# UBC-AWP/vision-sam3-yolo-lameless

Measured on AMD Instinct MI355X. Metric: frames/sec (whole node) for YOLO+SAM3+DINOv3 feature extraction, 1080p clips, higher is better.
Workload: dtype f16; 1 GPU; BASELINE cfg#5, dense schedule: fused per-frame path on a synthetic 5 s @ 30 fps 1080p clip (150 unique BGR frames resident in HBM): YOLOv8-l detect (letterbox 384x640, NMS, scale_boxes; f16 plan) -> SAM (Hiera-B+ image encoder + FPN at 1024x1024, box-prompted mask decoder, 1080p mask + statistics + contour features) + DINOv3 ViT-L/16 embed (224x224) on EVERY frame; per-frame records packed, gathe; parallelism=one clip per GPU, 1 GPU(s), one gather per step, streams=7

## Files before the change

### vision-sam3-yolo-lameless_amd/csrc/gemm.hip

```cpp
#include "common.h"
#include <stdlib.h>

namespace {

constexpr int BK = 64;

template <int BM, int BN, int AMODE, int OUT_DT>
__global__ __launch_bounds__(256, 2) void gemm_kernel(const lmx_gemm_desc p) {
  extern __shared__ __attribute__((aligned(16))) char smem[];
  half_t* As = reinterpret_cast<half_t*>(smem);
  half_t* Ws = As + 2 * BM * BK;
  constexpr int FM = BM / 32;
  constexpr int FN = BN / 32;
  constexpr int AI = BM / 32;
  constexpr int WI = BN / 32;

  const int tid = threadIdx.x;
  const int lane = tid & 63;
  const int wave = tid >> 6;
  const int wm = wave & 1, wn = wave >> 1;

  const int nwg = gridDim.x;
  const int bid = blockIdx.x;
  const int q = nwg >> 3, r = nwg & 7, xcd = bid & 7;
// ... 69 lines not shown
    half_t* as = As + buf * BM * BK;
    half_t* ws = Ws + buf * BN * BK;
#pragma unroll
    for (int i = 0; i < AI; ++i) {
      const int row = r0 + 32 * i;
      *reinterpret_cast<half8_t*>(as + row * BK + ((c ^ (row & 7)) << 3)) = a_st[i];
    }
#pragma unroll
    for (int i = 0; i < WI; ++i) {
      const int row = r0 + 32 * i;
      *reinterpret_cast<half8_t*>(ws + row * BK + ((c ^ (row & 7)) << 3)) = w_st[i];
    }
  };

  f32x4 acc[FM][FN];
#pragma unroll
  for (int i = 0; i < FM; ++i)
#pragma unroll
    for (int j = 0; j < FN; ++j) acc[i][j] = f32x4{0.f, 0.f, 0.f, 0.f};

  const int nk = (p.K + BK - 1) / BK;
  load_tile(0);
  store_tile(0);
  __syncthreads();

  const int frow = lane & 15;
  const int fq = lane >> 4;
  for (int kt = 0; kt < nk; ++kt) {
    const int buf = kt & 1;
    if (kt + 1 < nk) load_tile(kt + 1);
    const half_t* as = As + buf * BM * BK + (wm * (BM / 2) + frow) * BK;
    const half_t* ws = Ws + buf * BN * BK + (wn * (BN / 2) + frow) * BK;
#pragma unroll
    for (int ks = 0; ks < 2; ++ks) {
      const int coff = (((ks << 2) + fq) ^ (frow & 7)) << 3;
      half8_t af[FM], wf[FN];
#pragma unroll
      for (int i = 0; i < FM; ++i) af[i] = *reinterpret_cast<const half8_t*>(as + i * 16 * BK + coff);
#pragma unroll
      for (int j = 0; j < FN; ++j) wf[j] = *reinterpret_cast<const half8_t*>(ws + j * 16 * BK + coff);
#pragma unroll
      for (int i = 0; i < FM; ++i)
#pragma unroll
        for (int j = 0; j < FN; ++j)
          acc[i][j] = __builtin_amdgcn_mfma_f32_16x16x32_f16(wf[j], af[i], acc[i][j], 0, 0, 0);
    }
    if (kt + 1 < nk) store_tile(buf ^ 1);
    __syncthreads();
  }

  if (p.act == LMX_ACT_SWIGLU) {
    if constexpr (OUT_DT == LMX_F16 && FN % 2 == 0) {
      half_t* C = reinterpret_cast<half_t*>(p.C);
#pragma unroll
      for (int i = 0; i < FM; ++i) {
        const int m = m0 + wm * (BM / 2) + i * 16 + frow;
        if (m >= p.M) continue;
#pragma unroll
        for (int j = 0; j < FN; j += 2) {
          const int n = n0 + wn * (BN / 2) + j * 16 + fq * 4;
          if (n >= p.N) continue;
          f32x4 g = acc[i][j], u = acc[i][j + 1];
          if (p.bias) {
            g += *reinterpret_cast<const f32x4*>(p.bias + n);
            u += *reinterpret_cast<const f32x4*>(p.bias + n + 16);
          }
          const int no = (n >> 5) * 16 + (n & 15);
          f32x4 v;
#pragma unroll
          for (int e = 0; e < 4; ++e) v[e] = __fmul_rn(lmx_act(g[e], LMX_ACT_SILU), u[e]);
          if (p.scale) {
            const f32x4 s = *reinterpret_cast<const f32x4*>(p.scale + no);
#pragma unroll
            for (int e = 0; e < 4; ++e) v[e] = __fmul_rn(v[e], s[e]);
          }
          half4_t o;
#pragma unroll
          for (int e = 0; e < 4; ++e) o[e] = (half_t)v[e];
          *reinterpret_cast<half4_t*>(C + (int64_t)m * p.ldc + no) = o;
        }
      }
    }
    return;
  }

#pragma unroll
  for (int i = 0; i < FM; ++i) {
    const int m = m0 + wm * (BM / 2) + i * 16 + frow;
    if (m >= p.M) continue;
    const int mr = p.res_rows > 0 ? m % p.res_rows : m;
#pragma unroll
    for (int j = 0; j < FN; ++j) {
      const int n = n0 + wn * (BN / 2) + j * 16 + fq * 4;
      if (n >= p.N) continue;
      f32x4 v = acc[i][j];
      if (p.bias) {
        const f32x4 b = *reinterpret_cast<const f32x4*>(p.bias + n);
        v += b;
      }
      if (p.act != LMX_ACT_NONE) {
#pragma unroll
        for (int e = 0; e < 4; ++e) v[e] = lmx_act(v[e], p.act);
      }
      if (p.scale) {
        const f32x4 s = *reinterpret_cast<const f32x4*>(p.scale + n);
#pragma unroll
        for (int e = 0; e < 4; ++e) v[e] = __fmul_rn(v[e], s[e]);
      }
      if (OUT_DT == LMX_F32) {
        float* C = reinterpret_cast<float*>(p.C);
        if (p.res) {
          const f32x4 rr = *reinterpret_cast<const f32x4*>(reinterpret_cast<const float*>(p.res) + (int64_t)mr * p.ldr + n);
#pragma unroll
          for (int e = 0; e < 4; ++e) v[e] = __fadd_rn(v[e], rr[e]);
        }
        *reinterpret_cast<f32x4*>(C + (int64_t)m * p.ldc + n) = v;
      } else {
        half_t* C = reinterpret_cast<half_t*>(p.C);
        if (p.res) {
          const half4_t rr =
              *reinterpret_cast<const half4_t*>(reinterpret_cast<const half_t*>(p.res) + (int64_t)mr * p.ldr + n);
#pragma unroll
          for (int e = 0; e < 4; ++e) v[e] = __fadd_rn((float)(half_t)v[e], (float)rr[e]);
        }
        half4_t o;
#pragma unroll
        for (int e = 0; e < 4; ++e) o[e] = (half_t)v[e];
        *reinterpret_cast<half4_t*>(C + (int64_t)m * p.ldc + n) = o;
      }
    }
  }
}

template <int BM, int BN, int AMODE, int OUT_DT>
int launch(const lmx_gemm_desc& d, hipStream_t st) {
  const int MT = (d.M + BM - 1) / BM, NT = (d.N + BN - 1) / BN;
  const size_t smem = (size_t)2 * (BM + BN) * BK * sizeof(half_t);
  int dev;
  LMX_TRY(lmx_stream_device(st, &dev));
  LMX_TRY(lmx_allow_lds(reinterpret_cast<const void*>(&gemm_kernel<BM, BN, AMODE, OUT_DT>), (int)smem, dev));
  hipLaunchKernelGGL((gemm_kernel<BM, BN, AMODE, OUT_DT>), dim3(MT * NT), dim3(256), smem, st, d);
  return lmx_launch_check("gemm_kernel");
}

template <int AMODE, int OUT_DT>
int dispatch_tile(const lmx_gemm_desc& d, hipStream_t st) {
  if (d.N <= 64 || (d.N < 128 && d.N % 128 != 0)) return launch<128, 64, AMODE, OUT_DT>(d, st);
  return launch<128, 128, AMODE, OUT_DT>(d, st);
}

}

int lmx_gemm2_launch(const lmx_gemm_desc& d, hipStream_t st);

static bool force_v1() {
  static const int v = lmx_env_char("LMX_GEMM_V1");
  return v == '1';
}

extern "C" int lmx_k_gemm(const lmx_gemm_desc* dp, lmx_stream_t stream) {
  LMX_REQUIRE(dp != nullptr, "lmx_k_gemm: null descriptor");
  const lmx_gemm_desc& d = *dp;
  LMX_REQUIRE(d.A && d.W && d.C, "lmx_k_gemm: null A/W/C");
  LMX_REQUIRE(d.M > 0 && d.N > 0 && d.K > 0, "lmx_k_gemm: empty problem M=%d N=%d K=%d", d.M, d.N, d.K);
  LMX_REQUIRE(d.K % 8 == 0, "lmx_k_gemm: K=%d must be a multiple of 8", d.K);
  LMX_REQUIRE(d.N % 4 == 0, "lmx_k_gemm: N=%d must be a multiple of 4", d.N);
  LMX_REQUIRE(d.lda % 8 == 0, "lmx_k_gemm: lda=%lld must be a multiple of 8", (long long)d.lda);
  const bool gated = d.act == LMX_ACT_SWIGLU;
  LMX_REQUIRE(d.ldc % 4 == 0 && d.ldc >= (gated ? d.N / 2 : d.N), "lmx_k_gemm: bad ldc=%lld", (long long)d.ldc);
  LMX_REQUIRE(aligned16(d.A) && aligned16(d.W), "lmx_k_gemm: A/W must be 16-byte aligned");
  LMX_REQUIRE((((uintptr_t)d.C) & 7) == 0, "lmx_k_gemm: C must be 8-byte aligned");
  LMX_REQUIRE(d.out_dtype == LMX_F16 || d.out_dtype == LMX_F32, "lmx_k_gemm: bad out_dtype %d", d.out_dtype);
  LMX_REQUIRE(d.out_dtype == LMX_F16 || aligned16(d.C), "lmx_k_gemm: f32 C must be 16-byte aligned");
  LMX_REQUIRE(d.act >= LMX_ACT_NONE && d.act <= LMX_ACT_SWIGLU, "lmx_k_gemm: bad act %d", d.act);
  if (gated) {
    LMX_REQUIRE(d.N % 32 == 0, "lmx_k_gemm: LMX_ACT_SWIGLU: N=%d (gate + up rows, interleaved by 16) must be a multiple of 32", d.N);
    LMX_REQUIRE(!d.res, "lmx_k_gemm: LMX_ACT_SWIGLU takes no residual");
    LMX_REQUIRE(d.a_mode == 0 && d.a_rep <= 1 && d.split_k <= 1, "lmx_k_gemm: LMX_ACT_SWIGLU: dense A only (a_mode 0; no pooled rows, convolution, a_rep or split_k); a_mode=%d", d.a_mode);
    LMX_REQUIRE(d.out_dtype == LMX_F16, "lmx_k_gemm: LMX_ACT_SWIGLU writes f16 (one rounding of the f32 product)");
  }
  if (d.bias) LMX_REQUIRE(aligned16(d.bias), "lmx_k_gemm: bias must be 16-byte aligned");
  if (d.scale) LMX_REQUIRE(aligned16(d.scale), "lmx_k_gemm: scale must be 16-byte aligned");
  if (d.res) LMX_REQUIRE(d.ldr % 4 == 0 && d.ldr >= d.N, "lmx_k_gemm: bad ldr=%lld", (long long)d.ldr);
  LMX_REQUIRE(d.res_rows >= 0, "lmx_k_gemm: res_rows");
  if (d.a_mode == 0) {
    LMX_REQUIRE(d.a_rep > 1 || d.lda >= d.K, "lmx_k_gemm: lda=%lld < K=%d", (long long)d.lda, d.K);
  } else if (d.a_mode == 1) {
    LMX_REQUIRE(d.Cin > 0 && d.Cin % 8 == 0, "lmx_k_gemm: conv Cin=%d must be a multiple of 8", d.Cin);
    LMX_REQUIRE(d.K == 9 * d.Cin, "lmx_k_gemm: conv K=%d != 9*Cin=%d", d.K, 9 * d.Cin);
    LMX_REQUIRE(d.conv_stride == 1 || d.conv_stride == 2, "lmx_k_gemm: conv stride %d", d.conv_stride);
    LMX_REQUIRE(d.H > 0 && d.W_ > 0, "lmx_k_gemm: conv H/W");
    LMX_REQUIRE(d.Ho == (d.H + 2 - 3) / d.conv_stride + 1 && d.Wo == (d.W_ + 2 - 3) / d.conv_stride + 1,
                "lmx_k_gemm: conv Ho/Wo (%d,%d) inconsistent with H/W (%d,%d) stride %d", d.Ho, d.Wo, d.H, d.W_,
                d.conv_stride);
    LMX_REQUIRE(d.M % (d.Ho * d.Wo) == 0, "lmx_k_gemm: conv M=%d not a multiple of Ho*Wo", d.M);
    LMX_REQUIRE(d.lda >= d.Cin, "lmx_k_gemm: conv pixel stride lda=%lld < Cin=%d", (long long)d.lda, d.Cin);
  } else if (d.a_mode == 2) {
    LMX_REQUIRE(d.lda >= d.K, "lmx_k_gemm: lda=%lld < K=%d", (long long)d.lda, d.K);
    LMX_REQUIRE(d.H > 0 && d.W_ > 0 && d.H % 2 == 0 && d.W_ % 2 == 0 && d.M % (d.H * d.W_) == 0,
                "lmx_k_gemm: pooled rows need an even H x W token grid that divides M (H=%d W=%d M=%d)", d.H, d.W_, d.M);
    LMX_REQUIRE(!d.res && !d.scale && d.act == LMX_ACT_NONE, "lmx_k_gemm: pooled rows: no residual / scale / activation");
    LMX_REQUIRE(((int64_t)d.M * d.lda + d.K) * 2 < 0x7fffffffll, "lmx_k_gemm: pooled rows: A must be smaller than 2 GB");
    LMX_REQUIRE(d.M >= 512 && d.N >= 96 && d.N % 8 == 0 && d.ldc % 8 == 0 && aligned16(d.C),
                "lmx_k_gemm: pooled rows are built for the LDS-DMA kernel (M >= 512, N >= 96, N %% 8 == 0): use GEMM + maxpool2 for M=%d N=%d", d.M, d.N);
  } else {
    LMX_REQUIRE(false, "lmx_k_gemm: bad a_mode %d", d.a_mode);
  }
  LMX_REQUIRE(d.a_rep >= 0 && d.a_rep <= 3, "lmx_k_gemm: a_rep=%d (0..3)", d.a_rep);
  LMX_REQUIRE(d.split_k >= 0 && d.split_k <= 64, "lmx_k_gemm: split_k=%d (0..64)", d.split_k);
  if (d.split_k > 1) {
    LMX_REQUIRE(d.out_dtype == LMX_F32 && d.act == LMX_ACT_NONE && d.a_mode != 2 && d.a_rep <= 1, "lmx_k_gemm: split_k needs f32 output, no activation, a_mode 0 or 1");
    LMX_REQUIRE(d.split_stride >= (int64_t)(d.M - 1) * d.ldc + d.N && d.split_stride % 4 == 0, "lmx_k_gemm: split_stride=%lld", (long long)d.split_stride);
    LMX_REQUIRE((d.K + 63) / 64 >= d.split_k, "lmx_k_gemm: split_k=%d exceeds the k-tiles of K=%d", d.split_k, d.K);
    const bool conv_ok2 = d.a_mode == 1 && d.Cin % 32 == 0 && d.H < 32768 && d.W_ < 32768;
    LMX_REQUIRE((d.a_mode == 0 || conv_ok2) && d.N >= 64 && d.N % 8 == 0 && d.ldc % 8 == 0 && (!d.res || d.ldr % 8 == 0) &&
                    aligned16(d.C) && (!d.res || aligned16(d.res)),
                "lmx_k_gemm: split_k is built into the LDS-DMA kernel only (N >= 64, N %% 8 == 0; conv: Cin %% 32 == 0); M=%d N=%d", d.M, d.N);
    return lmx_gemm2_launch(d, reinterpret_cast<hipStream_t>(stream));
  }
  if (d.a_rep > 1) {
    LMX_REQUIRE(d.a_mode == 0 && d.K % d.a_rep == 0 && (d.K / d.a_rep) % 64 == 0, "lmx_k_gemm: a_rep=%d needs a_mode 0 and K / a_rep a multiple of 64 (K=%d)", d.a_rep, d.K);
    LMX_REQUIRE(d.lda >= d.K / d.a_rep, "lmx_k_gemm: lda=%lld < K / a_rep", (long long)d.lda);
    LMX_REQUIRE(d.M >= 512 && d.N >= 96 && d.N % 8 == 0 && d.ldc % 8 == 0 && (!d.res || d.ldr % 8 == 0) && aligned16(d.C) && (!d.res || aligned16(d.res)),
                "lmx_k_gemm: a_rep is built into the LDS-DMA kernel only (M >= 512, N >= 96, N %% 8 == 0); M=%d N=%d", d.M, d.N);
    return lmx_gemm2_launch(d, reinterpret_cast<hipStream_t>(stream));
  }
  hipStream_t st = reinterpret_cast<hipStream_t>(stream);
  const bool conv_ok = d.a_mode == 1 && d.Cin % 32 == 0 && d.H < 32768 && d.W_ < 32768;
  if (d.a_mode == 2) return lmx_gemm2_launch(d, st);
  static const int n64 = lmx_env_char("LMX_GEMM_N64") != '0';
  const int n_min = (conv_ok && n64 && d.M >= 65536) ? 64 : 96;
  if ((d.a_mode == 0 || conv_ok) && d.M >= 512 && d.N >= n_min && d.N % 8 == 0 && d.ldc % 8 == 0 && (!d.res || d.ldr % 8 == 0) &&
      aligned16(d.C) && (!d.res || aligned16(d.res)) && !force_v1())
    return lmx_gemm2_launch(d, st);
  if (d.a_mode == 0) {
    return d.out_dtype == LMX_F16 ? dispatch_tile<0, LMX_F16>(d, st) : dispatch_tile<0, LMX_F32>(d, st);
  }
  return d.out_dtype == LMX_F16 ? dispatch_tile<1, LMX_F16>(d, st) : dispatch_tile<1, LMX_F32>(d, st);
}
```

### vision-sam3-yolo-lameless_amd/csrc/gemm2.hip

```cpp
#include "common.h"
#include <stdlib.h>
#include <type_traits>

#ifdef LMX_DBG_TIMELINE
__device__ unsigned long long lmx_tl[8 * 16384];
extern "C" int lmx_dbg_get_timeline(void* host, int64_t bytes) { return (int)hipMemcpyFromSymbol(host, HIP_SYMBOL(lmx_tl), bytes); }
#define TL(i, v) if (threadIdx.x == 0 && swz < 16384) lmx_tl[swz * 8 + (i)] = (v)
#else
#define TL(i, v)
#endif
namespace lmx_gemm2 {

__device__ __forceinline__ float act_apply(float v, int act) { return lmx_act(v, act); }

constexpr int smem_bytes(int BM, int BN, int BK, int NSTAGE) { return NSTAGE * (BM + BN) * BK * 2 + 2 * BN * 4; }
constexpr int waves_per_simd(int BM, int BN, int BK, int NSTAGE) {
  const int smem = smem_bytes(BM, BN, BK, NSTAGE), nwave = (BM / 64) * (BN / 64);
  const int wps = (smem <= 80 * 1024 ? 2 : 1) * nwave / 4;
  return wps < 1 ? 1 : wps;
}
template <int OUT_DT, int BM, int BN, int BK, int NSTAGE, int AMODE, int STAG, bool GATED = false>
__global__ __launch_bounds__(waves_per_simd(BM, BN, BK, NSTAGE) * 256) void gemm2_kernel(const lmx_gemm_desc p, const int ntiles, const int nt_ok) {
  constexpr int NWAVE = (BM / 64) * (BN / 64);
  constexpr int STAGE_BYTES = (BM + BN) * BK * 2;
  constexpr int A_INSTR = BM * BK * 2 / 1024 / NWAVE;
  constexpr int W_INSTR = BN * BK * 2 / 1024 / NWAVE;
  constexpr int ROWS_PER_INSTR = 1024 / (BK * 2);
  constexpr int CHUNKS = BK / 8;
  constexpr int LA = NSTAGE - 1;
  extern __shared__ __attribute__((aligned(16))) char smem[];
  const int tid = threadIdx.x;
  const int lane = tid & 63;
  const int wave = __builtin_amdgcn_readfirstlane(tid >> 6);
  const int wm = wave % (BM / 64), wn = wave / (BM / 64);

  const int bid = blockIdx.x, xcd = bid & 7;
  const int q = ntiles >> 3, r = ntiles & 7;
  const int base = xcd < r ? xcd * (q + 1) : r * (q + 1) + (xcd - r) * q;
  const int cnt = q + (xcd < r ? 1 : 0);
  const int stride = ((int)gridDim.x + 7 - xcd) >> 3;
  const int NT = (p.N + BN - 1) / BN;
  for (int li = bid >> 3; li < cnt; li += stride) {
  const int swz = base + li;
  const int S_ = p.split_k > 1 ? p.split_k : 1;
  const int tile_ = swz / S_, sp_ = swz - tile_ * S_;
  const int mt = tile_ / NT, nt = tile_ - mt * NT;
  const int m0 = mt * BM, n0 = nt * BN;
  TL(0, (unsigned long long)__builtin_amdgcn_s_getreg((31 << 11) | 4));
  TL(1, (unsigned long long)__builtin_amdgcn_s_getreg((31 << 11) | 20));
  TL(2, wall_clock64());
  TL(5, (unsigned long long)bid);

  const int hw_out = (AMODE == 1) ? p.Ho * p.Wo : 1;
  const int img0 = (AMODE == 1) ? m0 / hw_out : 0;
  const char* Ab = reinterpret_cast<const char*>(p.A) +
                   ((AMODE == 1) ? (int64_t)img0 * p.H * p.W_ * p.lda * 2 : (AMODE == 2 ? (int64_t)0 : (int64_t)m0 * p.lda * 2));
  const char* Wb = reinterpret_cast<const char*>(p.W) + (int64_t)n0 * p.K * 2;
  const int Ka = (AMODE == 0 && p.a_rep > 1) ? p.K / p.a_rep : p.K;
  int64_t a_bytes = (AMODE == 1) ? ((int64_t)(p.M / hw_out - img0) * p.H * p.W_ - 1) * p.lda * 2 + (int64_t)p.Cin * 2
                                 : ((int64_t)(p.M - (AMODE == 2 ? 0 : m0) - 1) * p.lda + Ka) * 2;
  int64_t w_bytes = (int64_t)(p.N - n0) * p.K * 2;
  if (a_bytes > 0x7FFFFFF0ll) a_bytes = 0x7FFFFFF0ll;
  if (w_bytes > 0x7FFFFFF0ll) w_bytes = 0x7FFFFFF0ll;
  const __amdgpu_buffer_rsrc_t a_rs = __builtin_amdgcn_make_buffer_rsrc(const_cast<char*>(Ab), 0, (int)a_bytes, 0x00020000);
  const __amdgpu_buffer_rsrc_t w_rs = __builtin_amdgcn_make_buffer_rsrc(const_cast<char*>(Wb), 0, (int)w_bytes, 0x00020000);

  const int lrow = lane / CHUNKS;
  const int lsw = (BK == 64) ? (lrow & 7) : ((-(lrow >> 2)) & 3);
  const int lchunk = (lane % CHUNKS) ^ lsw;
  unsigned a_off[A_INSTR], w_off[W_INSTR];
  int a_yx[A_INSTR];
#pragma unroll
  for (int j = 0; j < A_INSTR; ++j) {
    const int row = (wave * A_INSTR + j) * ROWS_PER_INSTR + lrow;
    if (AMODE == 0) {
      a_off[j] = (unsigned)(row * (int)p.lda * 2 + lchunk * 16);
      a_yx[j] = 0;
    } else if (AMODE == 2) {
      const int m = m0 + row, g = m >> 2, sub = m & 3;
      const int Wq = p.W_ >> 1, gpi = (p.H >> 1) * Wq;
      const int img = g / gpi, rem = g - img * gpi;
      const int gy = rem / Wq, gx = rem - gy * Wq;
      const int tok = (img * p.H + 2 * gy + (sub >> 1)) * p.W_ + 2 * gx + (sub & 1);
      a_off[j] = m < p.M ? (unsigned)(tok * (int)p.lda * 2 + lchunk * 16) : 0x80000000u;
      a_yx[j] = 0;
    } else {
      const int m = m0 + row;
      const int img = m / hw_out, rem = m - img * hw_out;
      const int oy = rem / p.Wo, ox = rem - oy * p.Wo;
      const int iy0 = oy * p.conv_stride - 1, ix0 = ox * p.conv_stride - 1;
      a_off[j] = (unsigned)((((img - img0) * p.H + iy0) * p.W_ + ix0) * (int)p.lda * 2 + lchunk * 16);
      a_yx[j] = (m < p.M) ? ((iy0 << 16) | (ix0 & 0xffff)) : 0x80008000;
    }
  }
#pragma unroll
  for (int j = 0; j < W_INSTR; ++j)
    w_off[j] = (unsigned)(((wave * W_INSTR + j) * ROWS_PER_INSTR + lrow) * p.K * 2 + lchunk * 16);
  const unsigned OOB = 0x80000000u;
  const int nk = (p.K + BK - 1) / BK;
  const int nk64 = (p.K + 63) / 64;
  const int kt0 = (int)((int64_t)sp_ * nk64 / S_) * (64 / BK);
  const int kte = sp_ + 1 == S_ ? nk : (int)((int64_t)(sp_ + 1) * nk64 / S_) * (64 / BK);
  const int nloc = kte - kt0;
  const int nkA = (AMODE == 0 && p.a_rep > 1) ? nk / p.a_rep : nk;
  const bool k_tail_lane = (nk - 1) * BK + lchunk * 8 >= p.K;

  auto issue = [&](int kt, int slot) {
    char* st = smem + slot * STAGE_BYTES;
    const bool kill = (kt == nk - 1) && k_tail_lane;
    const int soff = kt * (BK * 2);
    if (AMODE != 1) {
      const int kta = kt - (kt >= nkA ? nkA : 0) - (kt >= 2 * nkA ? nkA : 0);
      const int soff_a = (AMODE == 0) ? kta * (BK * 2) : soff;
#pragma unroll
      for (int j = 0; j < A_INSTR; ++j) {
        char* dst = st + (wave * A_INSTR + j) * 1024;
        lds_dma16(a_rs, dst, kill ? OOB : a_off[j], soff_a);
      }
    } else {
      const int k0 = kt * BK;
      const int tap = k0 / p.Cin, ci0 = k0 - tap * p.Cin;
      const int ky = tap / 3, kx = tap - 3 * ky;
      const int tap_off = ((ky * p.W_ + kx) * (int)p.lda + ci0) * 2;
#pragma unroll
      for (int j = 0; j < A_INSTR; ++j) {
        char* dst = st + (wave * A_INSTR + j) * 1024;
        const int iy = (a_yx[j] >> 16) + ky, ix = (int)(short)(a_yx[j] & 0xffff) + kx;
        const bool ok = (unsigned)iy < (unsigned)p.H && (unsigned)ix < (unsigned)p.W_;
        lds_dma16(a_rs, dst, ok ? a_off[j] + (unsigned)tap_off : OOB, 0);
      }
    }
#pragma unroll
    for (int j = 0; j < W_INSTR; ++j) {
      char* dst = st + BM * BK * 2 + (wave * W_INSTR + j) * 1024;
      lds_dma16(w_rs, dst, kill ? OOB : w_off[j], soff);
    }
  };

  f32x4 acc[4][4];
#pragma unroll
  for (int i = 0; i < 4; ++i)
#pragma unroll
    for (int j = 0; j < 4; ++j) acc[i][j] = f32x4{0.f, 0.f, 0.f, 0.f};

  float* bl = reinterpret_cast<float*>(smem + NSTAGE * STAGE_BYTES);
  float bias_v = 0.f, scale_v = 1.f;
  if (AMODE != 1 && tid < BN && n0 + tid < p.N) {
    if (p.bias && sp_ == 0) bias_v = p.bias[n0 + tid];
    if constexpr (GATED) {
      if (p.scale && tid < BN / 2 && (n0 >> 1) + tid < (p.N >> 1)) scale_v = p.scale[(n0 >> 1) + tid];
    } else {
      if (p.scale) scale_v = p.scale[n0 + tid];
    }
  }

#pragma unroll
  for (int t = 0; t < LA; ++t)
    if (t < nloc) issue(kt0 + t, t);

  const int frow = lane & 15, fq = lane >> 4;
  const int fsw = (BK == 64) ? (frow & 7) : ((-(frow >> 2)) & 3);
  constexpr int PT = A_INSTR + W_INSTR;
  if constexpr (STAG == 0) {
  for (int kt = 0; kt < nloc; ++kt) {
    const int left = nloc - 1 - kt;
    wait_tiles<PT>(left < LA - 1 ? left : LA - 1);
    __builtin_amdgcn_s_barrier();
#ifdef LMX_DBG_TIMELINE
    if (kt == 0) { TL(6, wall_clock64()); }
    if (kt == 1) { TL(7, wall_clock64()); }
#endif
    if (kt + LA < nloc) issue(kt0 + kt + LA, (kt + LA) % NSTAGE);
    const char* st = smem + (kt % NSTAGE) * STAGE_BYTES;
    const half_t* as = reinterpret_cast<const half_t*>(st) + (wm * 64 + frow) * BK;
    const half_t* ws = reinterpret_cast<const half_t*>(st + BM * BK * 2) + (wn * 64 + frow) * BK;
#ifdef LMX_DBG_NOMFMA
    if (p.M < 0)
#endif
#pragma unroll
    for (int ks = 0; ks < BK / 32; ++ks) {
      const int coff = (((ks << 2) + fq) ^ fsw) << 3;
      half8_t af[4], wf[4];
#pragma unroll
      for (int j = 0; j < 4; ++j) wf[j] = *reinterpret_cast<const half8_t*>(ws + j * 16 * BK + coff);
#pragma unroll
      for (int i = 0; i < 4; ++i) af[i] = *reinterpret_cast<const half8_t*>(as + i * 16 * BK + coff);
      __builtin_amdgcn_s_setprio(1);
#pragma unroll
      for (int i = 0; i < 4; ++i)
#pragma unroll
        for (int j = 0; j < 4; ++j)
          acc[i][j] = __builtin_amdgcn_mfma_f32_16x16x32_f16(wf[j], af[i], acc[i][j], 0, 0, 0);
      __builtin_amdgcn_s_setprio(0);
    }
  }
  } else {
  const int grp = wave >= NWAVE / 2 ? 1 : 0;
  {
    const int y = nloc - 1 < LA - 1 ? nloc - 1 : LA - 1;
    wait_tiles<PT>(y);
  }
  __builtin_amdgcn_s_barrier();
  if (grp) __builtin_amdgcn_s_barrier();
  for (int kt = 0; kt < nloc; ++kt) {
    const char* st = smem + (kt % NSTAGE) * STAGE_BYTES;
    const half_t* as = reinterpret_cast<const half_t*>(st) + (wm * 64 + frow) * BK;
    const half_t* ws = reinterpret_cast<const half_t*>(st + BM * BK * 2) + (wn * 64 + frow) * BK;
    half8_t af[BK / 32][4], wf[BK / 32][4];
#pragma unroll
    for (int ks = 0; ks < BK / 32; ++ks) {
      const int coff = (((ks << 2) + fq) ^ fsw) << 3;
#pragma unroll
      for (int j = 0; j < 4; ++j) wf[ks][j] = *reinterpret_cast<const half8_t*>(ws + j * 16 * BK + coff);
#pragma unroll
      for (int i = 0; i < 4; ++i) af[ks][i] = *reinterpret_cast<const half8_t*>(as + i * 16 * BK + coff);
    }
    if (kt + 1 < nloc) {
      const int rest = nloc - 2 - kt;
      wait_tiles<PT>(rest < LA - 2 ? (rest < 0 ? 0 : rest) : (LA - 2 < 0 ? 0 : LA - 2));
    }
    if (kt + LA < nloc) issue(kt0 + kt + LA, (kt + LA) % NSTAGE);
    asm volatile("s_waitcnt lgkmcnt(0)" ::: "memory");
    __builtin_amdgcn_s_barrier();
    __builtin_amdgcn_s_setprio(1);
#pragma unroll
    for (int ks = 0; ks < BK / 32; ++ks)
#pragma unroll
      for (int i = 0; i < 4; ++i)
#pragma unroll
        for (int j = 0; j < 4; ++j)
          acc[i][j] = __builtin_amdgcn_mfma_f32_16x16x32_f16(wf[ks][j], af[ks][i], acc[i][j], 0, 0, 0);
    __builtin_amdgcn_s_setprio(0);
    __builtin_amdgcn_s_barrier();
  }
  if (!grp) __builtin_amdgcn_s_barrier();
  }

  if (AMODE == 1 && tid < BN && n0 + tid < p.N) {
    if (p.bias && sp_ == 0) bias_v = p.bias[n0 + tid];
    if (p.scale) scale_v = p.scale[n0 + tid];
  }
  if (tid < BN) {
    bl[tid] = bias_v;
    bl[BN + tid] = scale_v;
  }
  asm volatile("s_waitcnt lgkmcnt(0)" ::: "memory");
  __builtin_amdgcn_s_barrier();
  TL(3, wall_clock64());
#ifdef LMX_DBG_NOEPI
  if (p.M > 0 && acc[0][0][0] != 12345.f) continue;
#endif
  const bool nt_out = nt_ok && OUT_DT == LMX_F16 && ((p.ldc * 2) & 127) == 0 && (int64_t)p.M * p.N >= (16ll << 20);
  char* my = smem + wave * 4608;
  auto epilogue = [&](auto act_c, auto scale_c) {
    constexpr int ACT = decltype(act_c)::value;
    constexpr bool SCALE = decltype(scale_c)::value;
    const float* blj = bl + wn * 64 + fq * 4;
    auto finish = [&](f32x4 v, int j) -> f32x4 {
      v += *reinterpret_cast<const f32x4*>(blj + j * 16);
      if constexpr (ACT == LMX_ACT_GELU) {
        const f32x2 g0 = gelu_pk(f32x2{v[0], v[1]}), g1 = gelu_pk(f32x2{v[2], v[3]});
        v = f32x4{g0[0], g0[1], g1[0], g1[1]};
      } else if constexpr (ACT != LMX_ACT_NONE) {
#pragma unroll
        for (int e = 0; e < 4; ++e) v[e] = act_apply(v[e], ACT);
      }
      if constexpr (SCALE) v *= *reinterpret_cast<const f32x4*>(blj + BN + j * 16);
      return v;
    };
    if constexpr (ACT == LMX_ACT_SWIGLU) {
      if constexpr (OUT_DT == LMX_F16 && AMODE == 0) {
        half_t* t16 = reinterpret_cast<half_t*>(my);
        constexpr int RS = 40;
        const bool nt_g = nt_ok && ((p.ldc * 2) & 127) == 0 && (int64_t)p.M * p.N >= (32ll << 20);
#pragma unroll
        for (int pass = 0; pass < 2; ++pass) {
#pragma unroll
          for (int ii = 0; ii < 2; ++ii)
#pragma unroll
            for (int jj = 0; jj < 2; ++jj) {
              const f32x4 g = acc[pass * 2 + ii][2 * jj] + *reinterpret_cast<const f32x4*>(blj + jj * 32);
              const f32x4 u = acc[pass * 2 + ii][2 * jj + 1] + *reinterpret_cast<const f32x4*>(blj + jj * 32 + 16);
              f32x4 v;
#pragma unroll
              for (int e = 0; e < 4; ++e) v[e] = __fmul_rn(act_apply(g[e], LMX_ACT_SILU), u[e]);
              if constexpr (SCALE) {
                const f32x4 sc = *reinterpret_cast<const f32x4*>(bl + BN + wn * 32 + jj * 16 + fq * 4);
#pragma unroll
                for (int e = 0; e < 4; ++e) v[e] = __fmul_rn(v[e], sc[e]);
              }
              const half4_t o = {(half_t)v[0], (half_t)v[1], (half_t)v[2], (half_t)v[3]};
              *reinterpret_cast<half4_t*>(t16 + (ii * 16 + frow) * RS + jj * 16 + fq * 4) = o;
            }
#pragma unroll
          for (int it = 0; it < 2; ++it) {
            const int row = it * 16 + (lane >> 2), c8 = lane & 3;
            const half8_t o = *reinterpret_cast<const half8_t*>(t16 + row * RS + c8 * 8);
            const int m = m0 + wm * 64 + pass * 32 + row;
            const int no = ((n0 + wn * 64) >> 1) + c8 * 8;
            if (m < p.M && no < (p.N >> 1)) {
              half8_t* dst = reinterpret_cast<half8_t*>(reinterpret_cast<half_t*>(p.C) + (int64_t)m * p.ldc + no);
              if (nt_g)
                asm volatile("global_store_dwordx4 %0, %1, off nt" ::"v"(dst), "v"(o) : "memory");
              else
                *dst = o;
            }
          }
        }
      }
    } else if constexpr (OUT_DT == LMX_F16 && AMODE == 2) {
#pragma unroll
      for (int pass = 0; pass < 4; ++pass)
#pragma unroll
        for (int j = 0; j < 4; ++j) {
          f32x4 v = finish(acc[pass][j], j);
#pragma unroll
          for (int e = 0; e < 4; ++e) {
            v[e] = fmaxf(v[e], __shfl_xor(v[e], 1, 64));
            v[e] = fmaxf(v[e], __shfl_xor(v[e], 2, 64));
          }
          const int m = m0 + wm * 64 + pass * 16 + frow;
          const int n = n0 + wn * 64 + j * 16 + fq * 4;
          if ((frow & 3) == 0 && m < p.M && n < p.N)
            *reinterpret_cast<half4_t*>(reinterpret_cast<half_t*>(p.C) + (int64_t)(m >> 2) * p.ldc + n) =
                half4_t{(half_t)v[0], (half_t)v[1], (half_t)v[2], (half_t)v[3]};
          __builtin_amdgcn_sched_barrier(0);
        }
    } else if constexpr (OUT_DT == LMX_F16) {
      half_t* t16 = reinterpret_cast<half_t*>(my);
      constexpr int RS = 72;
#pragma unroll
      for (int pass = 0; pass < 2; ++pass) {
#pragma unroll
        for (int ii = 0; ii < 2; ++ii)
#pragma unroll
          for (int j = 0; j < 4; ++j) {
            const f32x4 v = finish(acc[pass * 2 + ii][j], j);
            const half4_t o = {(half_t)v[0], (half_t)v[1], (half_t)v[2], (half_t)v[3]};
            *reinterpret_cast<half4_t*>(t16 + (ii * 16 + frow) * RS + j * 16 + fq * 4) = o;
          }
#pragma unroll
        for (int it = 0; it < 4; ++it) {
          const int row = it * 8 + (lane >> 3), c8 = lane & 7;
          half8_t o = *reinterpret_cast<const half8_t*>(t16 + row * RS + c8 * 8);
          const int m = m0 + wm * 64 + pass * 32 + row;
          const int n = n0 + wn * 64 + c8 * 8;
          if (m < p.M && n < p.N) {
            if (p.res) {
              const int mr = p.res_rows > 0 ? m % p.res_rows : m;
              const half8_t rr = *reinterpret_cast<const half8_t*>(reinterpret_cast<const half_t*>(p.res) + (int64_t)mr * p.ldr + n);
#pragma unroll
              for (int e = 0; e < 8; ++e) o[e] = (half_t)((float)o[e] + (float)rr[e]);
            }
            half8_t* dst = reinterpret_cast<half8_t*>(reinterpret_cast<half_t*>(p.C) + (int64_t)m * p.ldc + n);
            if (nt_out)
              asm volatile("global_store_dwordx4 %0, %1, off nt" ::"v"(dst), "v"(o) : "memory");
            else
              *dst = o;
          }
        }
      }
    } else if constexpr (AMODE == 2) {
#pragma unroll
      for (int pass = 0; pass < 4; ++pass)
#pragma unroll
        for (int j = 0; j < 4; ++j) {
          f32x4 v = finish(acc[pass][j], j);
#pragma unroll
          for (int e = 0; e < 4; ++e) {
            v[e] = fmaxf(v[e], __shfl_xor(v[e], 1, 64));
            v[e] = fmaxf(v[e], __shfl_xor(v[e], 2, 64));
          }
          const int m = m0 + wm * 64 + pass * 16 + frow;
          const int n = n0 + wn * 64 + j * 16 + fq * 4;
          if ((frow & 3) == 0 && m < p.M && n < p.N) *reinterpret_cast<f32x4*>(reinterpret_cast<float*>(p.C) + (int64_t)(m >> 2) * p.ldc + n) = v;
          __builtin_amdgcn_sched_barrier(0);
        }
    } else {
      float* t32 = reinterpret_cast<float*>(my);
      constexpr int RS = 68;
      const int lrow = lane >> 4, c16 = lane & 15;
      const int n = n0 + wn * 64 + c16 * 4;
      const bool has_res = p.res != nullptr && sp_ == 0;
      float* Cs = reinterpret_cast<float*>(p.C) + (int64_t)sp_ * p.split_stride;
      f32x4 rr[4];
      auto load_res = [&](int pass) {
        f32x4* d = rr;
#pragma unroll
        for (int it = 0; it < 4; ++it) {
          const int m = m0 + wm * 64 + pass * 16 + it * 4 + lrow;
          d[it] = f32x4{0.f, 0.f, 0.f, 0.f};
          if (has_res && m < p.M && n < p.N) {
            const int mr = p.res_rows > 0 ? m % p.res_rows : m;
            d[it] = *reinterpret_cast<const f32x4*>(reinterpret_cast<const float*>(p.res) + (int64_t)mr * p.ldr + n);
          }
        }
      };
#pragma unroll
      for (int pass = 0; pass < 4; ++pass) {
        load_res(pass);
#pragma unroll
        for (int j = 0; j < 4; ++j) *reinterpret_cast<f32x4*>(t32 + frow * RS + j * 16 + fq * 4) = finish(acc[pass][j], j);
#pragma unroll
        for (int it = 0; it < 4; ++it) {
          const int row = it * 4 + lrow;
          f32x4 o = *reinterpret_cast<const f32x4*>(t32 + row * RS + c16 * 4);
          const int m = m0 + wm * 64 + pass * 16 + row;
          if (m < p.M && n < p.N) {
            if (has_res) o += rr[it];
            *reinterpret_cast<f32x4*>(Cs + (int64_t)m * p.ldc + n) = o;
          }
        }
      }
    }
  };
  {
    using T = std::true_type;
    using F = std::false_type;
    const int act = p.act;
    if constexpr (GATED) {
      if (p.scale) epilogue(std::integral_constant<int, LMX_ACT_SWIGLU>{}, T{});
      else epilogue(std::integral_constant<int, LMX_ACT_SWIGLU>{}, F{});
    } else if (p.scale) {
      if (act == LMX_ACT_NONE) epilogue(std::integral_constant<int, LMX_ACT_NONE>{}, T{});
      else if (act == LMX_ACT_SILU) epilogue(std::integral_constant<int, LMX_ACT_SILU>{}, T{});
      else if (act == LMX_ACT_GELU) epilogue(std::integral_constant<int, LMX_ACT_GELU>{}, T{});
      else epilogue(std::integral_constant<int, LMX_ACT_RELU>{}, T{});
    } else {
      if (act == LMX_ACT_NONE) epilogue(std::integral_constant<int, LMX_ACT_NONE>{}, F{});
      else if (act == LMX_ACT_SILU) epilogue(std::integral_constant<int, LMX_ACT_SILU>{}, F{});
      else if (act == LMX_ACT_GELU) epilogue(std::integral_constant<int, LMX_ACT_GELU>{}, F{});
      else epilogue(std::integral_constant<int, LMX_ACT_RELU>{}, F{});
    }
  }
  __builtin_amdgcn_s_barrier();
  TL(4, wall_clock64());
  }
}

template <int BM, int BN, int BK, int NSTAGE, int AMODE, int STAG = 0>
int launch2(const lmx_gemm_desc& d, hipStream_t st) {
  const int MT = (d.M + BM - 1) / BM, NT = (d.N + BN - 1) / BN;
  const size_t smem = smem_bytes(BM, BN, BK, NSTAGE);
  int dev;
  LMX_TRY(lmx_stream_device(st, &dev));
  LMX_TRY(lmx_allow_lds(reinterpret_cast<const void*>(&gemm2_kernel<LMX_F16, BM, BN, BK, NSTAGE, AMODE, STAG>), (int)smem, dev));
  LMX_TRY(lmx_allow_lds(reinterpret_cast<const void*>(&gemm2_kernel<LMX_F32, BM, BN, BK, NSTAGE, AMODE, STAG>), (int)smem, dev));
  const int ntiles = MT * NT * (d.split_k > 1 ? d.split_k : 1);
  int grid = ntiles;
  static const int persist = lmx_env_int("LMX_GEMM2_PERSIST", 0);
  static const int nt_ok = !lmx_env_set("LMX_GEMM2_NO_NT");
  if (persist > 0 && grid > 256 * persist) grid = 256 * persist;
  if (d.act == LMX_ACT_SWIGLU) {
    if constexpr (AMODE == 0) {
      LMX_TRY(lmx_allow_lds(reinterpret_cast<const void*>(&gemm2_kernel<LMX_F16, BM, BN, BK, NSTAGE, AMODE, STAG, true>), (int)smem, dev));
      hipLaunchKernelGGL((gemm2_kernel<LMX_F16, BM, BN, BK, NSTAGE, AMODE, STAG, true>), dim3(grid), dim3(BM * BN / 64), smem, st, d, ntiles, nt_ok);
      return lmx_launch_check("gemm2_kernel (gated)");
    } else {
      return LMX_EINVAL;
    }
  }
  if (d.out_dtype == LMX_F16)
    hipLaunchKernelGGL((gemm2_kernel<LMX_F16, BM, BN, BK, NSTAGE, AMODE, STAG>), dim3(grid), dim3(BM * BN / 64), smem, st, d, ntiles, nt_ok);
  else
    hipLaunchKernelGGL((gemm2_kernel<LMX_F32, BM, BN, BK, NSTAGE, AMODE, STAG>), dim3(grid), dim3(BM * BN / 64), smem, st, d, ntiles, nt_ok);
  return lmx_launch_check("gemm2_kernel");
}

}
using namespace lmx_gemm2;

static int g_variant = -1;
extern "C" void lmx_dbg_set_gemm2_variant(int v) { g_variant = v; }

int lmx_gemm2_launch(const lmx_gemm_desc& d, hipStream_t st) {
  if (g_variant < 0) g_variant = lmx_env_char("LMX_GEMM2_VARIANT");
  const int variant = g_variant;
  if (d.a_mode == 2) return launch2<256, 256, 64, 2, 2>(d, st);
  if (d.a_mode == 1) {
    static const int conv_small = lmx_env_set("LMX_GEMM2_CONV_SMALL");
    const int64_t t256 = (int64_t)((d.M + 255) / 256) * ((d.N + 255) / 256);
    const double q256 = (double)t256 / (double)(((t256 + 255) / 256) * 256);
    if (!conv_small && d.N % 256 == 0 && t256 >= 230 && q256 >= 0.75) return launch2<256, 256, 32, 3, 1, 1>(d, st);
    return launch2<256, 128, 32, 3, 1>(d, st);
  }
  switch (variant) {
    case 'A': return launch2<256, 128, 64, 3, 0>(d, st);
    case 'B': return launch2<128, 128, 64, 2, 0>(d, st);
    case 'C': return launch2<256, 128, 32, 3, 0>(d, st);
    case 'D': return launch2<256, 128, 32, 2, 0>(d, st);
    case 'E': return launch2<256, 256, 32, 3, 0>(d, st);
    case 'F': return launch2<256, 256, 32, 4, 0>(d, st);
    case 'H': return launch2<128, 128, 32, 2, 0>(d, st);
    case 'I': return launch2<128, 128, 32, 3, 0>(d, st);
    case 'S': return launch2<256, 128, 32, 6, 0, 1>(d, st);
    case 'T': return launch2<256, 128, 64, 3, 0, 1>(d, st);
    case 'U': return launch2<256, 128, 32, 3, 0, 1>(d, st);
    case 'V': return launch2<256, 128, 32, 4, 0, 1>(d, st);
    case 'W': return launch2<256, 256, 32, 4, 0, 1>(d, st);
    case 'Y': return launch2<256, 256, 32, 3, 0, 1>(d, st);
    case 'Z': return launch2<256, 256, 64, 2, 0>(d, st);
    default: {
      const int64_t nt256 = (d.N + 255) / 256, tiles256 = (int64_t)((d.M + 255) / 256) * nt256;
      const double nfrac = (double)d.N / (double)(nt256 * 256);
      const double q256 = (double)tiles256 / (double)(((tiles256 + 255) / 256) * 256);
      if (d.K >= 448 && tiles256 >= 200 && q256 >= 0.75 && nfrac >= 0.85) {
        return launch2<256, 256, 64, 2, 0>(d, st);
      }
      if (d.K < 448 && d.N >= 224 && d.N <= 1536 && d.N % 256 != 0 && nfrac >= 0.85 && tiles256 >= 200 && q256 >= 0.75)
        return d.K > 128 ? launch2<256, 256, 32, 3, 0>(d, st) : launch2<256, 256, 64, 2, 0>(d, st);
      const int64_t tiles = (int64_t)((d.M + 255) / 256) * ((d.N + 127) / 128);
      return (d.K >= 1792 || tiles <= 256) ? launch2<256, 128, 64, 3, 0, 1>(d, st) : launch2<256, 128, 32, 3, 0>(d, st);
    }
  }
}
```

Baseline: 683.2 frames/s.

## Add 256x224 GEMM tiling with configurable wave tiles for N divisible by 224

The LDS-DMA GEMM kernel now takes the per-wave tile size (WM x WN) as a template parameter. Load distribution, accumulator arrays, LDS slice sizing and the f16/f32 epilogues are generalised to match. A 256x224 block tile with 32x112 wave tiles is added and picked by default for dense GEMMs whose N is a multiple of 224 but not 256, with enough tiles and good wave quantisation. This targets padding waste in 256-wide N tiles for widths like 1792 or 4480, such as the ViT MLP layers. The cost is uneven W-load assignment across waves and a less-tuned wave shape. The diff also adds debug variants P/Q, and a forced variant now lowers the M>=512 threshold for routing to gemm2.

```diff
diff --git a/vision-sam3-yolo-lameless_amd/csrc/gemm.hip b/vision-sam3-yolo-lameless_amd/csrc/gemm.hip
--- a/vision-sam3-yolo-lameless_amd/csrc/gemm.hip
+++ b/vision-sam3-yolo-lameless_amd/csrc/gemm.hip
@@ -245,6 +245,7 @@
 }
 
 int lmx_gemm2_launch(const lmx_gemm_desc& d, hipStream_t st);
+bool lmx_gemm2_forced();
 
 static bool force_v1() {
   static const int v = lmx_env_char("LMX_GEMM_V1");
@@ -323,7 +324,8 @@
   if (d.a_mode == 2) return lmx_gemm2_launch(d, st);
   static const int n64 = lmx_env_char("LMX_GEMM_N64") != '0';
   const int n_min = (conv_ok && n64 && d.M >= 65536) ? 64 : 96;
-  if ((d.a_mode == 0 || conv_ok) && d.M >= 512 && d.N >= n_min && d.N % 8 == 0 && d.ldc % 8 == 0 && (!d.res || d.ldr % 8 == 0) &&
+  const int m_min = (d.a_mode == 0 && lmx_gemm2_forced()) ? 1 : 512;
+  if ((d.a_mode == 0 || conv_ok) && d.M >= m_min && d.N >= n_min && d.N % 8 == 0 && d.ldc % 8 == 0 && (!d.res || d.ldr % 8 == 0) &&
       aligned16(d.C) && (!d.res || aligned16(d.res)) && !force_v1())
     return lmx_gemm2_launch(d, st);
   if (d.a_mode == 0) {
diff --git a/vision-sam3-yolo-lameless_amd/csrc/gemm2.hip b/vision-sam3-yolo-lameless_amd/csrc/gemm2.hip
--- a/vision-sam3-yolo-lameless_amd/csrc/gemm2.hip
+++ b/vision-sam3-yolo-lameless_amd/csrc/gemm2.hip
@@ -14,25 +14,32 @@
 __device__ __forceinline__ float act_apply(float v, int act) { return lmx_act(v, act); }
 
 constexpr int smem_bytes(int BM, int BN, int BK, int NSTAGE) { return NSTAGE * (BM + BN) * BK * 2 + 2 * BN * 4; }
-constexpr int waves_per_simd(int BM, int BN, int BK, int NSTAGE) {
-  const int smem = smem_bytes(BM, BN, BK, NSTAGE), nwave = (BM / 64) * (BN / 64);
+constexpr int waves_per_simd(int BM, int BN, int BK, int NSTAGE, int WM = 64, int WN = 64) {
+  const int smem = smem_bytes(BM, BN, BK, NSTAGE), nwave = (BM / WM) * (BN / WN);
   const int wps = (smem <= 80 * 1024 ? 2 : 1) * nwave / 4;
   return wps < 1 ? 1 : wps;
 }
-template <int OUT_DT, int BM, int BN, int BK, int NSTAGE, int AMODE, int STAG, bool GATED = false>
-__global__ __launch_bounds__(waves_per_simd(BM, BN, BK, NSTAGE) * 256) void gemm2_kernel(const lmx_gemm_desc p, const int ntiles, const int nt_ok) {
-  constexpr int NWAVE = (BM / 64) * (BN / 64);
+template <int OUT_DT, int BM, int BN, int BK, int NSTAGE, int AMODE, int STAG, bool GATED = false, int WM = 64, int WN = 64>
+__global__ __launch_bounds__(waves_per_simd(BM, BN, BK, NSTAGE, WM, WN) * 256) void gemm2_kernel(const lmx_gemm_desc p, const int ntiles, const int nt_ok) {
+  constexpr int NWAVE = (BM / WM) * (BN / WN);
+  constexpr int FM = WM / 16, FN = WN / 16;
   constexpr int STAGE_BYTES = (BM + BN) * BK * 2;
   constexpr int A_INSTR = BM * BK * 2 / 1024 / NWAVE;
-  constexpr int W_INSTR = BN * BK * 2 / 1024 / NWAVE;
+  constexpr int W_PIECES = BN * BK * 2 / 1024;
+  constexpr int W_INSTR = (W_PIECES + NWAVE - 1) / NWAVE;
+  constexpr bool W_EVEN = W_PIECES % NWAVE == 0;
   constexpr int ROWS_PER_INSTR = 1024 / (BK * 2);
   constexpr int CHUNKS = BK / 8;
   constexpr int LA = NSTAGE - 1;
+  static_assert(BM % WM == 0 && BN % WN == 0 && WM % 32 == 0 && WN % 16 == 0 && (BM * BK * 2 / 1024) % NWAVE == 0 && (BN * BK * 2) % 1024 == 0,
+                "wave tiles cover the block tile; whole 1 KB pieces");
+  static_assert(W_EVEN || (LA == 1 && STAG == 0), "counted vmcnt waits assume the same number of LDS-DMAs on every wave");
+  static_assert((WM == 64 && WN == 64) || (AMODE == 0 && !GATED && STAG == 0), "other wave tiles: dense A, plain epilogues only");
   extern __shared__ __attribute__((aligned(16))) char smem[];
   const int tid = threadIdx.x;
   const int lane = tid & 63;
   const int wave = __builtin_amdgcn_readfirstlane(tid >> 6);
-  const int wm = wave % (BM / 64), wn = wave / (BM / 64);
+  const int wm = wave % (BM / WM), wn = wave / (BM / WM);
 
   const int bid = blockIdx.x, xcd = bid & 7;
   const int q = ntiles >> 3, r = ntiles & 7;
@@ -95,7 +102,7 @@
   }
 #pragma unroll
   for (int j = 0; j < W_INSTR; ++j)
-    w_off[j] = (unsigned)(((wave * W_INSTR + j) * ROWS_PER_INSTR + lrow) * p.K * 2 + lchunk * 16);
+    w_off[j] = (unsigned)(((W_EVEN ? wave * W_INSTR + j : j * NWAVE + wave) * ROWS_PER_INSTR + lrow) * p.K * 2 + lchunk * 16);
   const unsigned OOB = 0x80000000u;
   const int nk = (p.K + BK - 1) / BK;
   const int nk64 = (p.K + 63) / 64;
@@ -132,16 +139,16 @@
     }
 #pragma unroll
     for (int j = 0; j < W_INSTR; ++j) {
-      char* dst = st + BM * BK * 2 + (wave * W_INSTR + j) * 1024;
-      lds_dma16(w_rs, dst, kill ? OOB : w_off[j], soff);
+      const int piece = W_EVEN ? wave * W_INSTR + j : j * NWAVE + wave;
+      if (W_EVEN || piece < W_PIECES) lds_dma16(w_rs, st + BM * BK * 2 + piece * 1024, kill ? OOB : w_off[j], soff);
     }
   };
 
-  f32x4 acc[4][4];
-#pragma unroll
-  for (int i = 0; i < 4; ++i)
-#pragma unroll
-    for (int j = 0; j < 4; ++j) acc[i][j] = f32x4{0.f, 0.f, 0.f, 0.f};
+  f32x4 acc[FM][FN];
+#pragma unroll
+  for (int i = 0; i < FM; ++i)
+#pragma unroll
+    for (int j = 0; j < FN; ++j) acc[i][j] = f32x4{0.f, 0.f, 0.f, 0.f};
 
   float* bl = reinterpret_cast<float*>(smem + NSTAGE * STAGE_BYTES);
   float bias_v = 0.f, scale_v = 1.f;
@@ -172,24 +179,24 @@
 #endif
     if (kt + LA < nloc) issue(kt0 + kt + LA, (kt + LA) % NSTAGE);
     const char* st = smem + (kt % NSTAGE) * STAGE_BYTES;
-    const half_t* as = reinterpret_cast<const half_t*>(st) + (wm * 64 + frow) * BK;
-    const half_t* ws = reinterpret_cast<const half_t*>(st + BM * BK * 2) + (wn * 64 + frow) * BK;
+    const half_t* as = reinterpret_cast<const half_t*>(st) + (wm * WM + frow) * BK;
+    const half_t* ws = reinterpret_cast<const half_t*>(st + BM * BK * 2) + (wn * WN + frow) * BK;
 #ifdef LMX_DBG_NOMFMA
     if (p.M < 0)
 #endif
 #pragma unroll
     for (int ks = 0; ks < BK / 32; ++ks) {
       const int coff = (((ks << 2) + fq) ^ fsw) << 3;
-      half8_t af[4], wf[4];
-#pragma unroll
-      for (int j = 0; j < 4; ++j) wf[j] = *reinterpret_cast<const half8_t*>(ws + j * 16 * BK + coff);
-#pragma unroll
-      for (int i = 0; i < 4; ++i) af[i] = *reinterpret_cast<const half8_t*>(as + i * 16 * BK + coff);
+      half8_t af[FM], wf[FN];
+#pragma unroll
+      for (int j = 0; j < FN; ++j) wf[j] = *reinterpret_cast<const half8_t*>(ws + j * 16 * BK + coff);
+#pragma unroll
+      for (int i = 0; i < FM; ++i) af[i] = *reinterpret_cast<const half8_t*>(as + i * 16 * BK + coff);
       __builtin_amdgcn_s_setprio(1);
 #pragma unroll
-      for (int i = 0; i < 4; ++i)
-#pragma unroll
-        for (int j = 0; j < 4; ++j)
+      for (int i = 0; i < FM; ++i)
+#pragma unroll
+        for (int j = 0; j < FN; ++j)
           acc[i][j] = __builtin_amdgcn_mfma_f32_16x16x32_f16(wf[j], af[i], acc[i][j], 0, 0, 0);
       __builtin_amdgcn_s_setprio(0);
     }
@@ -204,8 +211,8 @@
   if (grp) __builtin_amdgcn_s_barrier();
   for (int kt = 0; kt < nloc; ++kt) {
     const char* st = smem + (kt % NSTAGE) * STAGE_BYTES;
-    const half_t* as = reinterpret_cast<const half_t*>(st) + (wm * 64 + frow) * BK;
-    const half_t* ws = reinterpret_cast<const half_t*>(st + BM * BK * 2) + (wn * 64 + frow) * BK;
+    const half_t* as = reinterpret_cast<const half_t*>(st) + (wm * WM + frow) * BK;
+    const half_t* ws = reinterpret_cast<const half_t*>(st + BM * BK * 2) + (wn * WN + frow) * BK;
     half8_t af[BK / 32][4], wf[BK / 32][4];
 #pragma unroll
     for (int ks = 0; ks < BK / 32; ++ks) {
@@ -251,11 +258,13 @@
   if (p.M > 0 && acc[0][0][0] != 12345.f) continue;
 #endif
   const bool nt_out = nt_ok && OUT_DT == LMX_F16 && ((p.ldc * 2) & 127) == 0 && (int64_t)p.M * p.N >= (16ll << 20);
-  char* my = smem + wave * 4608;
+  constexpr int SLICE = 32 * (WN + 8) * 2 > 16 * (WN + 4) * 4 ? 32 * (WN + 8) * 2 : 16 * (WN + 4) * 4;
+  static_assert(NWAVE * SLICE <= NSTAGE * STAGE_BYTES, "the epilogue slices lie inside the ring, below bias / scale");
+  char* my = smem + wave * SLICE;
   auto epilogue = [&](auto act_c, auto scale_c) {
     constexpr int ACT = decltype(act_c)::value;
     constexpr bool SCALE = decltype(scale_c)::value;
-    const float* blj = bl + wn * 64 + fq * 4;
+    const float* blj = bl + wn * WN + fq * 4;
     auto finish = [&](f32x4 v, int j) -> f32x4 {
       v += *reinterpret_cast<const f32x4*>(blj + j * 16);
       if constexpr (ACT == LMX_ACT_GELU) {
@@ -328,23 +337,25 @@
         }
     } else if constexpr (OUT_DT == LMX_F16) {
       half_t* t16 = reinterpret_cast<half_t*>(my);
-      constexpr int RS = 72;
-#pragma unroll
-      for (int pass = 0; pass < 2; ++pass) {
+      constexpr int RS = WN + 8;
+      constexpr int C8 = WN / 8;
+#pragma unroll
+      for (int pass = 0; pass < FM / 2; ++pass) {
 #pragma unroll
         for (int ii = 0; ii < 2; ++ii)
 #pragma unroll
-          for (int j = 0; j < 4; ++j) {
+          for (int j = 0; j < FN; ++j) {
             const f32x4 v = finish(acc[pass * 2 + ii][j], j);
             const half4_t o = {(half_t)v[0], (half_t)v[1], (half_t)v[2], (half_t)v[3]};
             *reinterpret_cast<half4_t*>(t16 + (ii * 16 + frow) * RS + j * 16 + fq * 4) = o;
           }
 #pragma unroll
-        for (int it = 0; it < 4; ++it) {
-          const int row = it * 8 + (lane >> 3), c8 = lane & 7;
+        for (int it = 0; it < C8 / 2; ++it) {
+          const int row = 64 % C8 == 0 ? it * (64 / C8) + lane / C8 : (it * 64 + lane) / C8;
+          const int c8 = 64 % C8 == 0 ? lane % C8 : (it * 64 + lane) % C8;
           half8_t o = *reinterpret_cast<const half8_t*>(t16 + row * RS + c8 * 8);
-          const int m = m0 + wm * 64 + pass * 32 + row;
-          const int n = n0 + wn * 64 + c8 * 8;
+          const int m = m0 + wm * WM + pass * 32 + row;
+          const int n = n0 + wn * WN + c8 * 8;
           if (m < p.M && n < p.N) {
             if (p.res) {
               const int mr = p.res_rows > 0 ? m % p.res_rows : m;
@@ -378,36 +389,43 @@
         }
     } else {
       float* t32 = reinterpret_cast<float*>(my);
-      constexpr int RS = 68;
-      const int lrow = lane >> 4, c16 = lane & 15;
-      const int n = n0 + wn * 64 + c16 * 4;
+      constexpr int RS = WN + 4;
+      constexpr int C4 = WN / 4;
+      constexpr bool WHOLE = 64 % C4 == 0;
+      const int lrow = lane / C4, lcol = lane % C4;
+      const int nl = n0 + wn * WN + lcol * 4;
+      auto prow = [&](int it) { return WHOLE ? it * (64 / C4) + lrow : (it * 64 + lane) / C4; };
+      auto pc = [&](int it) { return WHOLE ? lcol : (it * 64 + lane) % C4; };
+      auto pcol = [&](int it) { return WHOLE ? nl : n0 + wn * WN + pc(it) * 4; };
       const bool has_res = p.res != nullptr && sp_ == 0;
       float* Cs = reinterpret_cast<float*>(p.C) + (int64_t)sp_ * p.split_stride;
-      f32x4 rr[4];
-      auto load_res = [&](int pass) {
+      constexpr int NP = C4 / 4, RG = NP <= 4 ? NP : 4;
+      f32x4 rr[RG];
+      auto load_res = [&](int pass, int it0) {
         f32x4* d = rr;
 #pragma unroll
-        for (int it = 0; it < 4; ++it) {
-          const int m = m0 + wm * 64 + pass * 16 + it * 4 + lrow;
-          d[it] = f32x4{0.f, 0.f, 0.f, 0.f};
+        for (int it = it0; it < (it0 + RG < NP ? it0 + RG : NP); ++it) {
+          const int m = m0 + wm * WM + pass * 16 + prow(it), n = pcol(it);
+          d[it - it0] = f32x4{0.f, 0.f, 0.f, 0.f};
           if (has_res && m < p.M && n < p.N) {
             const int mr = p.res_rows > 0 ? m % p.res_rows : m;
-            d[it] = *reinterpret_cast<const f32x4*>(reinterpret_cast<const float*>(p.res) + (int64_t)mr * p.ldr + n);
+            d[it - it0] = *reinterpret_cast<const f32x4*>(reinterpret_cast<const float*>(p.res) + (int64_t)mr * p.ldr + n);
           }
         }
       };
 #pragma unroll
-      for (int pass = 0; pass < 4; ++pass) {
-        load_res(pass);
-#pragma unroll
-        for (int j = 0; j < 4; ++j) *reinterpret_cast<f32x4*>(t32 + frow * RS + j * 16 + fq * 4) = finish(acc[pass][j], j);
-#pragma unroll
-        for (int it = 0; it < 4; ++it) {
-          const int row = it * 4 + lrow;
-          f32x4 o = *reinterpret_cast<const f32x4*>(t32 + row * RS + c16 * 4);
-          const int m = m0 + wm * 64 + pass * 16 + row;
+      for (int pass = 0; pass < FM; ++pass) {
+        load_res(pass, 0);
+#pragma unroll
+        for (int j = 0; j < FN; ++j) *reinterpret_cast<f32x4*>(t32 + frow * RS + j * 16 + fq * 4) = finish(acc[pass][j], j);
+#pragma unroll
+        for (int it = 0; it < NP; ++it) {
+          if (it == RG) load_res(pass, RG);
+          const int row = prow(it), n = pcol(it);
+          f32x4 o = *reinterpret_cast<const f32x4*>(t32 + row * RS + pc(it) * 4);
+          const int m = m0 + wm * WM + pass * 16 + row;
           if (m < p.M && n < p.N) {
-            if (has_res) o += rr[it];
+            if (has_res) o += rr[it % RG];
             *reinterpret_cast<f32x4*>(Cs + (int64_t)m * p.ldc + n) = o;
           }
         }
@@ -438,32 +456,33 @@
   }
 }
 
-template <int BM, int BN, int BK, int NSTAGE, int AMODE, int STAG = 0>
+template <int BM, int BN, int BK, int NSTAGE, int AMODE, int STAG = 0, int WM = 64, int WN = 64>
 int launch2(const lmx_gemm_desc& d, hipStream_t st) {
+  constexpr int THREADS = (BM / WM) * (BN / WN) * 64;
   const int MT = (d.M + BM - 1) / BM, NT = (d.N + BN - 1) / BN;
   const size_t smem = smem_bytes(BM, BN, BK, NSTAGE);
   int dev;
   LMX_TRY(lmx_stream_device(st, &dev));
-  LMX_TRY(lmx_allow_lds(reinterpret_cast<const void*>(&gemm2_kernel<LMX_F16, BM, BN, BK, NSTAGE, AMODE, STAG>), (int)smem, dev));
-  LMX_TRY(lmx_allow_lds(reinterpret_cast<const void*>(&gemm2_kernel<LMX_F32, BM, BN, BK, NSTAGE, AMODE, STAG>), (int)smem, dev));
+  LMX_TRY(lmx_allow_lds(reinterpret_cast<const void*>(&gemm2_kernel<LMX_F16, BM, BN, BK, NSTAGE, AMODE, STAG, false, WM, WN>), (int)smem, dev));
+  LMX_TRY(lmx_allow_lds(reinterpret_cast<const void*>(&gemm2_kernel<LMX_F32, BM, BN, BK, NSTAGE, AMODE, STAG, false, WM, WN>), (int)smem, dev));
   const int ntiles = MT * NT * (d.split_k > 1 ? d.split_k : 1);
   int grid = ntiles;
   static const int persist = lmx_env_int("LMX_GEMM2_PERSIST", 0);
   static const int nt_ok = !lmx_env_set("LMX_GEMM2_NO_NT");
   if (persist > 0 && grid > 256 * persist) grid = 256 * persist;
   if (d.act == LMX_ACT_SWIGLU) {
-    if constexpr (AMODE == 0) {
+    if constexpr (AMODE == 0 && WM == 64 && WN == 64) {
       LMX_TRY(lmx_allow_lds(reinterpret_cast<const void*>(&gemm2_kernel<LMX_F16, BM, BN, BK, NSTAGE, AMODE, STAG, true>), (int)smem, dev));
-      hipLaunchKernelGGL((gemm2_kernel<LMX_F16, BM, BN, BK, NSTAGE, AMODE, STAG, true>), dim3(grid), dim3(BM * BN / 64), smem, st, d, ntiles, nt_ok);
+      hipLaunchKernelGGL((gemm2_kernel<LMX_F16, BM, BN, BK, NSTAGE, AMODE, STAG, true>), dim3(grid), dim3(THREADS), smem, st, d, ntiles, nt_ok);
       return lmx_launch_check("gemm2_kernel (gated)");
     } else {
       return LMX_EINVAL;
     }
   }
   if (d.out_dtype == LMX_F16)
-    hipLaunchKernelGGL((gemm2_kernel<LMX_F16, BM, BN, BK, NSTAGE, AMODE, STAG>), dim3(grid), dim3(BM * BN / 64), smem, st, d, ntiles, nt_ok);
+    hipLaunchKernelGGL((gemm2_kernel<LMX_F16, BM, BN, BK, NSTAGE, AMODE, STAG, false, WM, WN>), dim3(grid), dim3(THREADS), smem, st, d, ntiles, nt_ok);
   else
-    hipLaunchKernelGGL((gemm2_kernel<LMX_F32, BM, BN, BK, NSTAGE, AMODE, STAG>), dim3(grid), dim3(BM * BN / 64), smem, st, d, ntiles, nt_ok);
+    hipLaunchKernelGGL((gemm2_kernel<LMX_F32, BM, BN, BK, NSTAGE, AMODE, STAG, false, WM, WN>), dim3(grid), dim3(THREADS), smem, st, d, ntiles, nt_ok);
   return lmx_launch_check("gemm2_kernel");
 }
 
@@ -472,6 +491,10 @@
 
 static int g_variant = -1;
 extern "C" void lmx_dbg_set_gemm2_variant(int v) { g_variant = v; }
+bool lmx_gemm2_forced() {
+  if (g_variant < 0) g_variant = lmx_env_char("LMX_GEMM2_VARIANT");
+  return g_variant >= 'A' && g_variant <= 'Z';
+}
 
 int lmx_gemm2_launch(const lmx_gemm_desc& d, hipStream_t st) {
   if (g_variant < 0) g_variant = lmx_env_char("LMX_GEMM2_VARIANT");
@@ -500,10 +523,18 @@
     case 'W': return launch2<256, 256, 32, 4, 0, 1>(d, st);
     case 'Y': return launch2<256, 256, 32, 3, 0, 1>(d, st);
     case 'Z': return launch2<256, 256, 64, 2, 0>(d, st);
+    case 'P':
+    case 'Q':
+      LMX_REQUIRE(d.act != LMX_ACT_SWIGLU, "lmx_k_gemm: the 256 x 224 tiling has no gated (LMX_ACT_SWIGLU) epilogue");
+      return variant == 'P' ? launch2<256, 224, 64, 2, 0, 0, 32, 112>(d, st) : launch2<256, 224, 64, 2, 0, 0, 64, 112>(d, st);
     default: {
       const int64_t nt256 = (d.N + 255) / 256, tiles256 = (int64_t)((d.M + 255) / 256) * nt256;
       const double nfrac = (double)d.N / (double)(nt256 * 256);
       const double q256 = (double)tiles256 / (double)(((tiles256 + 255) / 256) * 256);
+      const int64_t tiles224 = (int64_t)((d.M + 255) / 256) * (d.N / 224);
+      const double q224 = (double)tiles224 / (double)(((tiles224 + 255) / 256) * 256);
+      if (d.act != LMX_ACT_SWIGLU && d.N % 224 == 0 && d.N % 256 != 0 && d.K >= 448 && tiles224 >= 200 && q224 >= 0.75)
+        return launch2<256, 224, 64, 2, 0, 0, 32, 112>(d, st);
       if (d.K >= 448 && tiles256 >= 200 && q256 >= 0.75 && nfrac >= 0.85) {
         return launch2<256, 256, 64, 2, 0>(d, st);
       }
```

Result: slower. 658.3 frames/s (-3.6%).
